# endernewton/tf-faster-rcnn

Measured on AMD Instinct MI355X. Metric: images/sec (600×1000) ResNet-101 Faster R-CNN at 1/2/4/8 MI355X, higher is better.
Workload: dtype f32 (operands, accumulators, results; GEMMs with Cin, Cout % 128 == 0 form each f32 product from two-piece fp16 operands with an exact power-of-two scale per 128-k block on the fp16 matrix pipe -- 3 MFMAs / product, dropped terms <= 3 * 2^-22, measured error vs float64 below the f32-MFMA kernel's; o

## Files before the change

tf-faster-rcnn_amd/csrc/gemm_h2.hip:

```cpp
#include "h2_common.h"
#include <mutex>
#include <type_traits>

typedef float f32x16 __attribute__((ext_vector_type(16)));
typedef _Float16 h8 __attribute__((ext_vector_type(8)));

#define LDS_AS __attribute__((address_space(3)))

struct GemmH2Params {
  const unsigned short* x; const float* x_inv; const unsigned short* w; const float* w_inv;
  const float* bias; const float* res; const unsigned short* resp; const float* resp_inv; float* y; unsigned short* yp; float* y_inv;
  int M, N, K, batch, act, nsteps, mtiles, ntiles;
  long long Mtot;
  int wshare;
  const float* mask;
  float* mean_part; int mean_rows;
#ifdef FRCNN_H2_TRACE
  unsigned long long* trace;
#endif
};

__device__ __forceinline__ void h2_glds16(unsigned voff, const void* sbase, unsigned lds_base) {
  unsigned keep;
  asm volatile(
// ... 12 lines not shown
  asm volatile(
      "s_mov_b32 %0, m0\n\t"
      "s_mov_b32 m0, %3\n\t"
      "s_nop 0\n\t"
      "global_load_lds_dword %1, %2\n\t"
      "s_mov_b32 m0, %0"
      : "=&s"(keep)
      : "v"(voff), "s"(sbase), "s"(lds_base)
      : "memory");
}

__device__ __forceinline__ void h2_glds16c(unsigned voff, const void* sbase, unsigned lds_base) {
  asm volatile(
      "s_mov_b32 m0, %2\n\t"
      "s_nop 0\n\t"
      "global_load_lds_dwordx4 %0, %1"
      :
      : "v"(voff), "s"(sbase), "s"(lds_base)
      : "memory");
}
__device__ __forceinline__ void h2_glds4c(unsigned voff, const void* sbase, unsigned lds_base) {
  asm volatile(
      "s_mov_b32 m0, %2\n\t"
      "s_nop 0\n\t"
      "global_load_lds_dword %0, %1"
      :
      : "v"(voff), "s"(sbase), "s"(lds_base)
      : "memory");
}

template <int N>
__device__ __forceinline__ void h2_wait_vmcnt() {
  asm volatile("s_waitcnt vmcnt(%0)" ::"n"(N) : "memory");
}

template <int BM, int BN, int WM, int WN, int NS, int WPE = 2, int TUNE = 0>
__global__ __launch_bounds__((BM / WM) * (BN / WN) * 64) __attribute__((amdgpu_waves_per_eu(WPE))) void k_gemm_h2(const GemmH2Params p) {
  constexpr int NW = (BM / WM) * (BN / WN);
  constexpr int TM = WM / 32, TN = WN / 32;
  constexpr int LA = 2 * BM / 16 / NW;
  constexpr int LB = 2 * BN / 16 / NW;
  constexpr int G = LA + LB;
  constexpr int SL = BM / 64;
  constexpr int XP = BM * 64, WP = BN * 64;
  constexpr bool PP = (TUNE & 32) != 0;
  constexpr bool LTB = (TUNE & 256) != 0;
  constexpr bool W21 = (TUNE & 512) != 0;
  constexpr bool DE = (TUNE & 1024) != 0;
  constexpr int NTA = (TUNE & 16384) ? 2 : 0;
  constexpr int S_OFF = 2 * XP + 2 * WP, STAGE = S_OFF + (PP ? 0 : 1024);
  constexpr int RED_OFF = NS * STAGE;
  constexpr int S2_OFF = RED_OFF + (BN / WN) * BM * 4;
  constexpr int CB_OFF = S2_OFF + (PP ? NW * 512 : (TUNE & 2) ? 2048 : 0);
  static_assert(!LTB || (!PP && NS == 2 && NW >= 3 && BN % 64 == 0), "light boundary: the two-slot one-barrier-per-slab schedule");
  static_assert(!DE || (LTB && W21 && BN == H2_KB), "deferred epilogue: built on the light boundary's LDS constants and counted waits");
  static_assert(!PP || (NW == 8 && NS == 3 && (TUNE & 2) && ((BM == 256 && WM == 64) || (BM == 128 && WM == 32)) && BN == 128 && WN == 64),
                "ping-pong geometry: 8 waves as 4 (M) x 2 (N), waves 0-3 = the upper half of the rows");
  static_assert((2 * BM / 16) % NW == 0 && (2 * BN / 16) % NW == 0, "tile/wave mismatch");
  static_assert(BM <= 256 && NS >= 2 && NS <= 4, "stage layout");
  static_assert((NS - 2) * (G + SL) <= 63, "vmcnt range");
  extern __shared__ __attribute__((aligned(16))) char smem[];

  const int tid = threadIdx.x, lane = tid & 63;
  const int wave = __builtin_amdgcn_readfirstlane(tid >> 6);
  const int per = p.mtiles * p.ntiles, T = per * p.batch;
  const int xcd = blockIdx.x & 7, wx = blockIdx.x >> 3, W8 = gridDim.x >> 3;
  const int tq = T / 8, tr = T % 8, tn = tq + (xcd < tr ? 1 : 0);
  const int t_end = (xcd < tr ? xcd * (tq + 1) : tr * (tq + 1) + (xcd - tr) * tq) + tn;
  const int tile0 = t_end - tn + wx;
  if (tile0 >= t_end) return;
  const int my_tiles = (t_end - tile0 + W8 - 1) / W8;
  int left = __builtin_amdgcn_readfirstlane(my_tiles * p.nsteps);

  const int wmi = wave / (BN / WN), wni = wave % (BN / WN);
  const int wm0 = wmi * WM, wn0 = wni * WN;
  const int frow = lane & 31, khalf = lane >> 5;

  const size_t xplane = (size_t)p.Mtot * p.K * 2, wplane = (size_t)p.N * p.K * 2;
  unsigned a_off[LA], b_off[LB], s_off[SL];
  const char* i_xb = nullptr; const char* i_wb = nullptr; const char* i_sb = nullptr;
  int i_tile = tile0, i_step = 0, i_par = 0, c_par = 0;
  int i_g = 0, i_bn0 = 0, i_cpar = 0, c_cpar = 0;
  int pend = 0;
#pragma unroll
  for (int t = 0; t < LB; ++t) {
    const int u = wave * LB + t, plane = u / (BN / 16), row = (u % (BN / 16)) * 16 + (lane >> 2), pos = lane & 3;
    b_off[t] = (unsigned)((size_t)plane * wplane + (size_t)row * p.K * 2 + ((pos ^ ((row >> ((TUNE & 8) ? 1 : 2)) & 3)) * 16));
// ... 212 lines not shown
#pragma unroll
      for (int i = 0; i < TM; ++i)
#pragma unroll
        for (int j = 0; j < TN; ++j) {
          tmp[i][j] = __builtin_amdgcn_mfma_f32_32x32x16_f16(wh[j], xl[i], tmp[i][j], 0, 0, 0);
          after(t * 3 * TM * TN + 2 * TM * TN + i * TN + j);
        }
    }
  };

  int c_tile = tile0, c_step = 0, cur = 0, nxt = 0;
  int c_bm0 = 0, c_bn0 = 0, c_g = 0;
  auto set_ctile = [&](int tl) {
    int g, mt, nt;
    tile_coords(tl, g, mt, nt);
    c_bm0 = mt * BM; c_bn0 = nt * BN; c_g = g;
  };
  const float act_lo = p.act == FRCNN_ACT_NONE ? -__builtin_inff() : 0.f;
  const float act_hi = p.act == FRCNN_ACT_RELU6 ? 6.f : __builtin_inff();

  auto rsrc_f = [&](const void* base, long long elems_left, int esize) {
    const long long bytes = elems_left * esize;
    return __builtin_amdgcn_make_buffer_rsrc((void*)base, 0, (int)max(0ll, min(bytes, 0x7fffffffll)), 0x00020000);
  };

  struct TileRef { int bm0, bn0, g, cpar; };
  auto ent_rsrc = [&](const void* base, int g, int esize) {
    const char* b = (const char*)base + (size_t)g * p.M * p.N * esize;
    return __builtin_amdgcn_make_buffer_rsrc((void*)b, 0, p.M * p.N * esize, 0x00020000);
  };
  const int lo4 = (frow * p.N + 4 * khalf) * 4;
  auto lo2_of = [&]() { int v = lo4; asm volatile("" : "+v"(v)); return v >> 1; };
  auto lo2w_of = [&]() { int v = lo4; asm volatile("" : "+v"(v)); return (v >> 1) + 8 * (int)(threadIdx.x >> 5 & 1); };
  auto sub_off = [&](const auto& T, int i, int j) {
    return __builtin_amdgcn_readfirstlane((T.bm0 + wm0 + i * 32) * p.N + T.bn0 + wn0 + j * 32);
  };

#ifdef FRCNN_H2_TRACE
  int tr_slab = 0;
  auto stamp = [&](int point) {
    if (p.trace && blockIdx.x < 16 && tr_slab < 64 && lane == 0)
      p.trace[(((size_t)blockIdx.x * NW + wave) * 64 + tr_slab) * 8 + point] = __builtin_amdgcn_s_memtime();
  };
  int tr_tile = 0;
  auto bstamp = [&](int point) {
    if (p.trace && blockIdx.x < 16 && tr_tile < 32 && lane == 0)
      p.trace[(size_t)16 * 8 * 64 * 8 + (((size_t)blockIdx.x * NW + wave) * 32 + tr_tile) * 8 + point] = __builtin_amdgcn_s_memtime();
  };
#else
  auto stamp = [](int) {};
  auto bstamp = [](int) {};
#endif
  float rri[TM];
  (void)rri;
  auto load_res_raw = [&](int i) {
    typedef unsigned u32x4 __attribute__((ext_vector_type(4)));
    const TileRef C{c_bm0, c_bn0, c_g, c_cpar};
    const bool planes = !p.res && p.resp;
    const auto none = __builtin_amdgcn_make_buffer_rsrc((void*)nullptr, 0, 0, 0x00020000);
    const auto r_even = p.res ? ent_rsrc(p.res, c_g, 4) : planes ? ent_rsrc(p.resp, c_g, 2) : none;
    const auto r_odd = p.res ? r_even : planes ? ent_rsrc(p.resp + (size_t)p.Mtot * p.N, c_g, 2) : none;
    const int step_q = planes ? 0 : 32, step_p = planes ? 32 : 0;
    int base = lo4;
    asm volatile("" : "+v"(base));
    if (planes) base = (base >> 1) + 8 * (int)(threadIdx.x >> 5 & 1);
#pragma unroll
    for (int j = 0; j < TN; ++j) {
      const int vo = base + sub_off(C, i, j) * (planes ? 2 : 4);
#pragma unroll
      for (int q = 0; q < 4; ++q) {
        const u32x4 ld = __builtin_amdgcn_raw_buffer_load_b128((q & 1) ? r_odd : r_even, vo, q * step_q + (q >> 1) * step_p, NTA);
        tot[i][j][4 * q + 0] = __uint_as_float(ld[0]); tot[i][j][4 * q + 1] = __uint_as_float(ld[1]);
        tot[i][j][4 * q + 2] = __uint_as_float(ld[2]); tot[i][j][4 * q + 3] = __uint_as_float(ld[3]);
      }
      pend += 4;
    }
    if (p.resp) rri[i] = p.resp_inv[(size_t)(c_bn0 / H2_KB) * p.Mtot + (size_t)c_g * p.M + min(c_bm0 + wm0 + i * 32 + frow, p.M - 1)];
  };
  auto init_tot = [&]() {
    if constexpr (DE) return;
    const size_t row_base = (size_t)c_g * p.M;
    typedef unsigned u32x4 __attribute__((ext_vector_type(4)));
    if (p.res) {
#pragma unroll
      for (int i = 0; i < TM; ++i)
#pragma unroll
        for (int j = 0; j < TN; ++j) {
          const int m0 = c_bm0 + wm0 + i * 32, nc = c_bn0 + wn0 + j * 32;
          const auto rr = rsrc_f(p.res + (long long)(row_base + m0) * p.N + nc, (long long)(p.M - m0) * p.N - nc, 4);
#pragma unroll
          for (int q = 0; q < 4; ++q) {
            const u32x4 ld = __builtin_amdgcn_raw_buffer_load_b128(rr, (frow * p.N + 4 * khalf) * 4 + 32 * q, 0, 0);
            tot[i][j][4 * q + 0] = __uint_as_float(ld[0]); tot[i][j][4 * q + 1] = __uint_as_float(ld[1]);
            tot[i][j][4 * q + 2] = __uint_as_float(ld[2]); tot[i][j][4 * q + 3] = __uint_as_float(ld[3]);
          }
        }
      pend += TM * TN * 4;
    } else if (p.resp) {
      float ri[TM];
#pragma unroll
      for (int i = 0; i < TM; ++i)
        ri[i] = p.resp_inv[(size_t)(c_bn0 / H2_KB) * p.Mtot + row_base + min(c_bm0 + wm0 + i * 32 + frow, p.M - 1)];
      h4 hv[TM][TN][4], lv[TM][TN][4];
#pragma unroll
      for (int i = 0; i < TM; ++i)
#pragma unroll
        for (int j = 0; j < TN; ++j) {
          const int m0 = c_bm0 + wm0 + i * 32, nc = c_bn0 + wn0 + j * 32;
          const long long sbase = (long long)(row_base + m0) * p.N + nc, left_e = (long long)(p.M - m0) * p.N - nc;
          const auto rh = rsrc_f(p.resp + sbase, left_e, 2), rl = rsrc_f(p.resp + (size_t)p.Mtot * p.N + sbase, left_e, 2);
// ... 60 lines not shown
      const int n0 = T.bn0 + wn0 + j * 32 + 4 * khalf;
#pragma unroll
      for (int q = 0; q < 4; ++q) {
        const float4 wi = LTB ? *(const float4*)(smem + CB_OFF + T.cpar * (2 * BN * 4) + (wn0 + j * 32 + 4 * khalf + 8 * q) * 4)
                             : *(const float4*)(p.w_inv + (size_t)(p.wshare ? 0 : T.g) * p.N + n0 + 8 * q);
#pragma unroll
        for (int i = 0; i < TM; ++i) {
          tot[i][j][4 * q + 0] = act_clamp(tot[i][j][4 * q + 0] * wi.x, act_lo, act_hi);
          tot[i][j][4 * q + 1] = act_clamp(tot[i][j][4 * q + 1] * wi.y, act_lo, act_hi);
          tot[i][j][4 * q + 2] = act_clamp(tot[i][j][4 * q + 2] * wi.z, act_lo, act_hi);
          tot[i][j][4 * q + 3] = act_clamp(tot[i][j][4 * q + 3] * wi.w, act_lo, act_hi);
        }
      }
    }
  };
  auto ep_mask = [&](const TileRef& T) {
    if ((TUNE & 128) && p.mask) {
      const auto rk = ent_rsrc(p.mask, T.g, 4);
#pragma unroll
      for (int i = 0; i < TM; ++i)
#pragma unroll
        for (int j = 0; j < TN; ++j) {
          const int vo = lo4 + sub_off(T, i, j) * 4;
          typedef unsigned u32x4 __attribute__((ext_vector_type(4)));
          u32x4 k[4];
#pragma unroll
          for (int q = 0; q < 4; ++q) k[q] = __builtin_amdgcn_raw_buffer_load_b128(rk, vo + 32 * q, 0, 0);
#pragma unroll
          for (int q = 0; q < 4; ++q)
#pragma unroll
            for (int e = 0; e < 4; ++e) tot[i][j][4 * q + e] = __uint_as_float(k[q][e]) > 0.f ? tot[i][j][4 * q + e] : 0.f;
        }
      pend += TM * TN * 4;
    }
  };
  auto ep_mean = [&](const TileRef& T) {
    const int nblk = (p.M + 31) >> 5;
#pragma unroll
    for (int i = 0; i < TM; ++i) {
      const int mb = T.bm0 + wm0 + i * 32;
      if (mb >= p.M) continue;
      const int m = mb + frow, g0 = mb / p.mean_rows, gid = m / p.mean_rows;
      const bool in_a = m < p.M && gid == g0, in_b = m < p.M && gid == g0 + 1;
      float* dst = p.mean_part + ((size_t)T.g * nblk + (mb >> 5)) * 2 * p.N;
#pragma unroll
      for (int j = 0; j < TN; ++j) {
        const int n0 = T.bn0 + wn0 + j * 32 + 4 * khalf;
#pragma unroll
        for (int q = 0; q < 4; ++q) {
          float a[4], b[4];
#pragma unroll
          for (int e = 0; e < 4; ++e) {
            const float v = tot[i][j][4 * q + e];
            a[e] = in_a ? v : 0.f;
            b[e] = in_b ? v : 0.f;
          }
#pragma unroll
          for (int o = 1; o < 32; o <<= 1)
#pragma unroll
            for (int e = 0; e < 4; ++e) {
              a[e] += __shfl_xor(a[e], o, 64);
              b[e] += __shfl_xor(b[e], o, 64);
            }
          if (frow == 0) {
            *(float4*)(dst + n0 + 8 * q) = make_float4(a[0], a[1], a[2], a[3]);
            *(float4*)(dst + p.N + n0 + 8 * q) = make_float4(b[0], b[1], b[2], b[3]);
          }
          pend += 2;
        }
      }
    }
  };
  auto ep_store_f32 = [&](const TileRef& T, int i) {
    if (!p.y) return;
    const auto ry = ent_rsrc(p.y, T.g, 4);
#pragma unroll
    for (int j = 0; j < TN; ++j) {
      const int lo = lo4 + sub_off(T, i, j) * 4;
#pragma unroll
      for (int q = 0; q < 4; ++q) {
        typedef unsigned u32x4 __attribute__((ext_vector_type(4)));
        u32x4 o;
        o[0] = __float_as_uint(tot[i][j][4 * q + 0]); o[1] = __float_as_uint(tot[i][j][4 * q + 1]);
        o[2] = __float_as_uint(tot[i][j][4 * q + 2]); o[3] = __float_as_uint(tot[i][j][4 * q + 3]);
        __builtin_amdgcn_raw_buffer_store_b128(o, ry, lo + 32 * q, 0, NTA);
      }
      pend += 4;
      if constexpr (DE) __builtin_amdgcn_sched_barrier(0);
    }
  };
  auto ep_rowmax_write = [&](float (&mx)[TM]) {
    float* red = (float*)(smem + RED_OFF);
#pragma unroll
    for (int i = 0; i < TM; ++i) {
      float m = 0.f;
#pragma unroll
      for (int j = 0; j < TN; ++j)
#pragma unroll
        for (int r = 0; r < 16; ++r) m = fmaxf(m, fabsf(tot[i][j][r]));
      m = fmaxf(m, __shfl_xor(m, 32, 64));
      mx[i] = m;
      if (BN / WN > 1 && khalf == 0) red[wni * BM + wm0 + i * 32 + frow] = m;
    }
  };
  auto ep_rowmax_merge = [&](float (&mx)[TM]) {
    const float* red = (const float*)(smem + RED_OFF);
#pragma unroll
    for (int i = 0; i < TM; ++i)
#pragma unroll
      for (int o = 0; o < BN / WN; ++o) mx[i] = fmaxf(mx[i], red[o * BM + wm0 + i * 32 + frow]);
  };
  auto ep_store_planes = [&](const TileRef& T, int i, float mxi) {
    const size_t row_base = (size_t)T.g * p.M;
    const size_t yplane = (size_t)p.Mtot * p.N;
    float scale, inv;
    h2_block_scale(mxi, scale, inv);
    const int m0 = T.bm0 + wm0 + i * 32;
    if (wni == 0 && khalf == 0 && m0 + frow < p.M)
      p.y_inv[(size_t)(T.bn0 / H2_KB) * p.Mtot + row_base + m0 + frow] = inv;
    const auto rh = ent_rsrc(p.yp, T.g, 2), rl = ent_rsrc(p.yp + yplane, T.g, 2);
#pragma unroll
    for (int j = 0; j < TN; ++j) {
      const int so = sub_off(T, i, j) * 2;
      typedef unsigned u32x2 __attribute__((ext_vector_type(2)));
      if constexpr (W21) {
        const int lo = lo2w_of() + so;
#pragma unroll
        for (int pq = 0; pq < 2; ++pq) {
          h4 ha, la, hb, lb;
          h2_split4(make_float4(tot[i][j][8 * pq + 0], tot[i][j][8 * pq + 1], tot[i][j][8 * pq + 2], tot[i][j][8 * pq + 3]), scale, ha, la);
          h2_split4(make_float4(tot[i][j][8 * pq + 4], tot[i][j][8 * pq + 5], tot[i][j][8 * pq + 6], tot[i][j][8 * pq + 7]), scale, hb, lb);
          const u32x2 uha = __builtin_bit_cast(u32x2, ha), uhb = __builtin_bit_cast(u32x2, hb);
          const u32x2 ula = __builtin_bit_cast(u32x2, la), ulb = __builtin_bit_cast(u32x2, lb);
          typedef unsigned u32x4 __attribute__((ext_vector_type(4)));
          const auto h0 = __builtin_amdgcn_permlane32_swap(uha[0], uhb[0], false, false), h1 = __builtin_amdgcn_permlane32_swap(uha[1], uhb[1], false, false);
          const auto l0 = __builtin_amdgcn_permlane32_swap(ula[0], ulb[0], false, false), l1 = __builtin_amdgcn_permlane32_swap(ula[1], ulb[1], false, false);
          __builtin_amdgcn_raw_buffer_store_b128(u32x4{h0[0], h1[0], h0[1], h1[1]}, rh, lo + 32 * pq, 0, NTA);
          __builtin_amdgcn_raw_buffer_store_b128(u32x4{l0[0], l1[0], l0[1], l1[1]}, rl, lo + 32 * pq, 0, NTA);
        }
        pend += 4;
        if constexpr (DE) __builtin_amdgcn_sched_barrier(0);
      } else {
        const int lo = lo2_of() + so;
#pragma unroll
        for (int q = 0; q < 4; ++q) {
          h4 hh, ll;
          h2_split4(make_float4(tot[i][j][4 * q + 0], tot[i][j][4 * q + 1], tot[i][j][4 * q + 2], tot[i][j][4 * q + 3]), scale, hh, ll);
          __builtin_amdgcn_raw_buffer_store_b64(__builtin_bit_cast(u32x2, hh), rh, lo + 16 * q, 0, 0);
          __builtin_amdgcn_raw_buffer_store_b64(__builtin_bit_cast(u32x2, ll), rl, lo + 16 * q, 0, 0);
        }
        pend += 8;
      }
// ... 20 lines not shown
      if (BN / WN > 1) {
        asm volatile("s_waitcnt lgkmcnt(0)" ::: "memory");
        __builtin_amdgcn_s_barrier();
        ep_rowmax_merge(mx);
      }
      bstamp(3);
#pragma unroll
      for (int i = 0; i < TM; ++i) ep_store_planes(T, i, mx[i]);
      bstamp(4);
      if (BN / WN > 1) {
        asm volatile("s_waitcnt lgkmcnt(0)" ::: "memory");
        __builtin_amdgcn_s_barrier();
      }
    }
    bstamp(5);
    c_cpar ^= 1;
  };

  constexpr int HALF = (TM + 1) / 2;
  bool have_prev = false;
  TileRef P{0, 0, 0, 0};
  float dmx[TM];
  (void)dmx;
  auto de_piece = [&](auto pos_c) {
    constexpr int POS = decltype(pos_c)::value;
    if constexpr (POS == 0) {
      if (have_prev) {
        ep_scale_act(P);
        ep_mask(P);
        if (p.yp) ep_rowmax_write(dmx);
      }
    } else if constexpr (POS == 1 || POS == 2) {
      constexpr int I0 = POS == 1 ? 0 : HALF, I1 = POS == 1 ? HALF : TM;
      if (have_prev) {
        if (POS == 1 && p.yp && BN / WN > 1) ep_rowmax_merge(dmx);
#pragma unroll
        for (int i = I0; i < I1; ++i) {
          ep_store_f32(P, i);
          if (p.yp) ep_store_planes(P, i, dmx[i]);
        }
      }
#pragma unroll
      for (int i = I0; i < I1; ++i) load_res_raw(i);
    }
  };

  auto slab = [&](auto pos_c, bool fold, bool first_block) {
    constexpr int POS = decltype(pos_c)::value;
    const std::integral_constant<bool, POS == 0> first_c{};
    stamp(0);
    if constexpr (DE) asm volatile("s_waitcnt lgkmcnt(0)" ::: "memory");
    if constexpr (LTB) {
      wait_pending(pend);
    } else if (left >= 1) {
      if (wave == 0) h2_wait_vmcnt<(NS - 2) * (G + SL)>(); else h2_wait_vmcnt<(NS - 2) * G>();
    } else {
      h2_wait_vmcnt<0>();
    }
    stamp(1);
    __builtin_amdgcn_s_barrier();
    stamp(2);
    const bool more = left > 0;
    constexpr int HALF = NO_LOAD ? 0 : (TUNE & 4) ? 0 : (TUNE & 1) ? (G + SL) / 2 : G + SL;
    static_assert(!LTB || NO_LOAD || HALF == G + SL, "light boundary: the slab's loads are issued in one burst");
    if (more) {
#pragma unroll
      for (int t = 0; t < HALF; ++t) issue_one(nxt, t);
      if constexpr (LTB) {
        if (i_step == 0) issue_cb();
        pend = 0;
      }
    }
    stamp(3);
    if constexpr (DE) {
      __builtin_amdgcn_sched_barrier(0);
      if (first_block) de_piece(pos_c);
      __builtin_amdgcn_sched_barrier(0);
    }
    float ainv[TM];
    if (fold) {
      const int soff = (TUNE & 2) ? S2_OFF + c_par * 1024 : cur * STAGE + S_OFF;
#pragma unroll
      for (int i = 0; i < TM; ++i) ainv[i] = *(const float*)(smem + soff + (wm0 + i * 32 + frow) * 4);
      c_par ^= 1;
    }
    if (!(TUNE & 4)) {
      slab_mfma(cur, first_c, [&]() {
        stamp(4);
        if (more && !NO_LOAD) {
#pragma unroll
          for (int t = HALF; t < G + SL; ++t) issue_one(nxt, t);
        }
      }, [](int) {});
    } else if (more) {
      slab_mfma(cur, first_c, []() {}, [&](int m) {
#pragma unroll
        for (int d = 0; d < ND; ++d)
          if (1 + (d * (NM - 1)) / ND == m) issue_one(nxt, d);
      });
    } else {
      slab_mfma(cur, first_c, []() {}, [](int) {});
    }
    stamp(5);
    if (more) {
      issue_advance();
      nxt = nxt + 1 == NS ? 0 : nxt + 1;
    }
    if (fold) {
      if (LTB && first_block) {
        const float* cbp = (const float*)(smem + CB_OFF + c_cpar * (2 * BN * 4));
        if (DE && !p.res && p.resp) {
          typedef unsigned u32x2 __attribute__((ext_vector_type(2)));
#pragma unroll
          for (int i = 0; i < TM; ++i)
#pragma unroll
            for (int j = 0; j < TN; ++j)
#pragma unroll
              for (int pq = 0; pq < 2; ++pq) {
                unsigned w[8];
#pragma unroll
                for (int e = 0; e < 8; ++e) w[e] = __float_as_uint(tot[i][j][8 * pq + e]);
                const auto h0 = __builtin_amdgcn_permlane32_swap(w[0], w[2], false, false), h1 = __builtin_amdgcn_permlane32_swap(w[1], w[3], false, false);
                const auto l0 = __builtin_amdgcn_permlane32_swap(w[4], w[6], false, false), l1 = __builtin_amdgcn_permlane32_swap(w[5], w[7], false, false);
                const h4 ha = __builtin_bit_cast(h4, u32x2{h0[0], h1[0]}), hb = __builtin_bit_cast(h4, u32x2{h0[1], h1[1]});
                const h4 la = __builtin_bit_cast(h4, u32x2{l0[0], l1[0]}), lb = __builtin_bit_cast(h4, u32x2{l0[1], l1[1]});
#pragma unroll
                for (int e = 0; e < 4; ++e) {
                  tot[i][j][8 * pq + e] = ((float)ha[e] + (float)la[e]) * rri[i];
                  tot[i][j][8 * pq + 4 + e] = ((float)hb[e] + (float)lb[e]) * rri[i];
                }
              }
        }
#pragma unroll
        for (int j = 0; j < TN; ++j)
#pragma unroll
          for (int q = 0; q < 4; ++q) {
            const float4 wi = *(const float4*)(cbp + wn0 + j * 32 + 4 * khalf + 8 * q);
            const float4 bv = p.bias ? *(const float4*)(cbp + BN + wn0 + j * 32 + 4 * khalf + 8 * q) : make_float4(0.f, 0.f, 0.f, 0.f);
            const float s0 = __uint_as_float(0x7f000000u - __float_as_uint(wi.x)), s1 = __uint_as_float(0x7f000000u - __float_as_uint(wi.y));
            const float s2 = __uint_as_float(0x7f000000u - __float_as_uint(wi.z)), s3 = __uint_as_float(0x7f000000u - __float_as_uint(wi.w));
#pragma unroll
            for (int i = 0; i < TM; ++i) {
              tot[i][j][4 * q + 0] = __builtin_fmaf(tmp[i][j][4 * q + 0], ainv[i], (tot[i][j][4 * q + 0] + bv.x) * s0);
              tot[i][j][4 * q + 1] = __builtin_fmaf(tmp[i][j][4 * q + 1], ainv[i], (tot[i][j][4 * q + 1] + bv.y) * s1);
              tot[i][j][4 * q + 2] = __builtin_fmaf(tmp[i][j][4 * q + 2], ainv[i], (tot[i][j][4 * q + 2] + bv.z) * s2);
              tot[i][j][4 * q + 3] = __builtin_fmaf(tmp[i][j][4 * q + 3], ainv[i], (tot[i][j][4 * q + 3] + bv.w) * s3);
            }
          }
      } else {
#pragma unroll
        for (int i = 0; i < TM; ++i)
#pragma unroll
          for (int j = 0; j < TN; ++j)
#pragma unroll
            for (int r = 0; r < 16; ++r) tot[i][j][r] = __builtin_fmaf(tmp[i][j][r], ainv[i], tot[i][j][r]);
      }
    }
    cur = cur + 1 == NS ? 0 : cur + 1;
    stamp(6);
#ifdef FRCNN_H2_TRACE
    ++tr_slab;
#endif
  };

  set_tile(i_tile);
  set_ctile(c_tile);
  if constexpr (PP) {
    const int grp = wave >> 2;
    h8 fxh[2][TM], fxl[2][TM], fwh[2][TN], fwl[2][TN];
    auto seg_barrier = [&]() {
      __builtin_amdgcn_sched_barrier(0);
      __builtin_amdgcn_s_barrier();
      __builtin_amdgcn_sched_barrier(0);
    };
    auto fold = [&]() {
      float ainv[TM];
#pragma unroll
      for (int i = 0; i < TM; ++i) ainv[i] = *(const float*)(smem + S2_OFF + (wave * 2 + c_par) * 256 + (i * 32 + frow) * 4);
      c_par ^= 1;
#pragma unroll
      for (int i = 0; i < TM; ++i)
#pragma unroll
        for (int j = 0; j < TN; ++j)
#pragma unroll
          for (int r = 0; r < 16; ++r) tot[i][j][r] = __builtin_fmaf(tmp[i][j][r], ainv[i], tot[i][j][r]);
    };
    auto pp_mem = [&](auto pos_c, bool fold_prev) -> bool {
      constexpr int POS = decltype(pos_c)::value;
      const char* sb = smem + cur * STAGE;
      stamp(0);
#pragma unroll
      for (int t = 0; t < 2; ++t) {
#pragma unroll
        for (int j = 0; j < TN; ++j) {
          const char* q = sb + w_row + j * 32 * 64 + (((2 * t + khalf) ^ sw) * 16);
          fwh[t][j] = __builtin_bit_cast(h8, *(const uint4*)(q));
          fwl[t][j] = __builtin_bit_cast(h8, *(const uint4*)(q + WP));
        }
#pragma unroll
        for (int i = 0; i < TM; ++i) {
          const char* q = sb + x_row + i * 32 * 64 + (((2 * t + khalf) ^ sw) * 16);
          fxh[t][i] = __builtin_bit_cast(h8, *(const uint4*)(q));
          fxl[t][i] = __builtin_bit_cast(h8, *(const uint4*)(q + XP));
        }
      }
      const bool more = left > 0;
      if (more) {
#pragma unroll
        for (int t = 0; t <= G; ++t) issue_one(nxt, t);
        issue_advance();
        nxt = nxt + 1 == NS ? 0 : nxt + 1;
      }
      if (fold_prev) fold();
      stamp(1);
      if (grp == 1) {
        if (more) h2_wait_vmcnt<(POS == 2 ? G + 1 : G)>(); else h2_wait_vmcnt<0>();
      }
      asm volatile("s_waitcnt lgkmcnt(0)" ::: "memory");
      stamp(2);
      seg_barrier();
      stamp(3);
      return more;
    };
    auto pp_mfma = [&](auto pos_c, bool issued) {
      constexpr int POS = decltype(pos_c)::value;
      __builtin_amdgcn_s_setprio(1);
#pragma unroll
      for (int t = 0; t < 2; ++t) {
#pragma unroll
        for (int i = 0; i < TM; ++i)
#pragma unroll
          for (int j = 0; j < TN; ++j) {
            if (POS == 0 && t == 0) {
              f32x16 z;
#pragma unroll
              for (int r = 0; r < 16; ++r) z[r] = 0.f;
              tmp[i][j] = __builtin_amdgcn_mfma_f32_32x32x16_f16(fwh[t][j], fxh[t][i], z, 0, 0, 0);
            } else {
              tmp[i][j] = __builtin_amdgcn_mfma_f32_32x32x16_f16(fwh[t][j], fxh[t][i], tmp[i][j], 0, 0, 0);
            }
          }
#pragma unroll
        for (int i = 0; i < TM; ++i)
#pragma unroll
          for (int j = 0; j < TN; ++j) tmp[i][j] = __builtin_amdgcn_mfma_f32_32x32x16_f16(fwl[t][j], fxh[t][i], tmp[i][j], 0, 0, 0);
#pragma unroll
        for (int i = 0; i < TM; ++i)
#pragma unroll
          for (int j = 0; j < TN; ++j) tmp[i][j] = __builtin_amdgcn_mfma_f32_32x32x16_f16(fwh[t][j], fxl[t][i], tmp[i][j], 0, 0, 0);
      }
      __builtin_amdgcn_s_setprio(0);
      stamp(4);
      if (grp == 0) {
        if (issued) h2_wait_vmcnt<(POS == 2 ? G + 1 : G)>(); else h2_wait_vmcnt<0>();
      }
      cur = cur + 1 == NS ? 0 : cur + 1;
      stamp(5);
      seg_barrier();
      stamp(6);
#ifdef FRCNN_H2_TRACE
      ++tr_slab;
#endif
    };
    bool two = false;
#pragma unroll
    for (int s2 = 0; s2 < 2; ++s2) {
      if (left > 0) {
#pragma unroll
        for (int t = 0; t <= G; ++t) issue_one(nxt, t);
        issue_advance();
        nxt = nxt + 1 == NS ? 0 : nxt + 1;
        two = s2 == 1;
      }
    }
    if (two) h2_wait_vmcnt<G>(); else h2_wait_vmcnt<0>();
    seg_barrier();
    if (grp == 1) seg_barrier();
    const int nkb = p.nsteps >> 2;
    for (int tl = 0; tl < my_tiles; ++tl) {
      init_tot();
      for (int kb = 0; kb < nkb; ++kb) {
        bool is;
        is = pp_mem(std::integral_constant<int, 0>{}, kb > 0); pp_mfma(std::integral_constant<int, 0>{}, is);
        is = pp_mem(std::integral_constant<int, 1>{}, false);  pp_mfma(std::integral_constant<int, 1>{}, is);
        is = pp_mem(std::integral_constant<int, 2>{}, false);  pp_mfma(std::integral_constant<int, 2>{}, is);
        is = pp_mem(std::integral_constant<int, 3>{}, false);  pp_mfma(std::integral_constant<int, 3>{}, is);
      }
      fold();
      epilogue();
      c_tile += W8;
      if (tl + 1 < my_tiles) set_ctile(c_tile);
    }
    if (grp == 0) seg_barrier();
    h2_wait_vmcnt<0>();
    return;
  }
#pragma unroll
  for (int s = 0; s < NS - 1; ++s) {
    if (left > 0) {
#pragma unroll
      for (int t = 0; t < G + SL; ++t) issue_one(nxt, t);
      if constexpr (LTB) {
        if (i_step == 0) issue_cb();
        pend = 0;
      }
      issue_advance();
      nxt = nxt + 1 == NS ? 0 : nxt + 1;
    }
  }
  const int nkb = p.nsteps >> 2;
  for (int tl = 0; tl < my_tiles; ++tl) {
    init_tot();
    bstamp(6);
#ifdef FRCNN_H2_TRACE
    ++tr_tile;
#endif
    for (int kb = 0; kb < nkb; ++kb) {
      slab(std::integral_constant<int, 0>{}, false, kb == 0);
      slab(std::integral_constant<int, 1>{}, false, kb == 0);
      slab(std::integral_constant<int, 2>{}, false, kb == 0);
      slab(std::integral_constant<int, 3>{}, true, kb == 0);
// ... 73 lines not shown
unsigned long long* g_h2_trace = nullptr;
extern "C" void frcnn_h2_set_trace(unsigned long long* buf) { g_h2_trace = buf; }
#endif

extern "C" size_t frcnn_h2_planes_bytes(long long rows, int K) {
  if (rows <= 0 || K <= 0) return 0;
  return (size_t)2 * (size_t)rows * (size_t)K * sizeof(unsigned short);
}

extern "C" int frcnn_h2_pack_w(const float* w_d, int G, int N, int K, void* planes_d, float* w_inv_d, void* stream) {
  if (!w_d || !planes_d || !w_inv_d || G <= 0 || N <= 0 || K <= 0) return FRCNN_E_ARG;
  if (K % 4) return FRCNN_E_UNSUPPORTED;
  const int rows = G * N;
  hipLaunchKernelGGL(k_h2_pack_w, dim3((unsigned)cdiv(rows, 4)), dim3(256), 0, (hipStream_t)stream, w_d, rows, N, K, (unsigned short*)planes_d, w_inv_d);
  LAUNCH_CHECK();
  return FRCNN_OK;
}

extern "C" int frcnn_h2_split(const float* x_d, long long M, int K, void* planes_d, float* inv_d, void* stream) {
  if (!x_d || !planes_d || !inv_d || M <= 0 || K <= 0) return FRCNN_E_ARG;
  if (K % H2_KB) return FRCNN_E_UNSUPPORTED;
  const long long pairs = M * (K / H2_KB);
  const unsigned grid = (unsigned)min((pairs + 7) / 8, (long long)256 * 64);
  hipLaunchKernelGGL(k_h2_split, dim3(grid), dim3(256), 0, (hipStream_t)stream, x_d, M, K, (unsigned short*)planes_d, inv_d);
  LAUNCH_CHECK();
  return FRCNN_OK;
}

template <int BM, int BN, int WM, int WN, int NS, int WPE = 2, int TUNE = 0>
static int launch_h2(const GemmH2Params& q, hipStream_t st) {
  constexpr int NT = (BM / WM) * (BN / WN) * 64;
  constexpr size_t lds = ((TUNE & 32) ? (size_t)NS * (2 * BM * 64 + 2 * BN * 64) + (size_t)(BN / WN) * BM * 4 + (size_t)(NT / 64) * 512
                                      : (size_t)NS * (2 * BM * 64 + 2 * BN * 64 + 1024) + (size_t)(BN / WN) * BM * 4 + ((TUNE & 2) ? 2048 : 0)) +
                         ((TUNE & 256) ? (size_t)2 * 2 * BN * 4 : 0);
  auto kern = k_gemm_h2<BM, BN, WM, WN, NS, WPE, TUNE>;
  static KernelOnce once;
  int slots = 0;
  HIP_TRY(kernel_once(once, (const void*)kern, NT, lds, &slots));
  if (slots < 8 || q.N % BN) return FRCNN_E_UNSUPPORTED;
  if (q.yp && BN != H2_KB) return FRCNN_E_UNSUPPORTED;
  GemmH2Params p = q;
  p.mtiles = cdiv(p.M, BM); p.ntiles = p.N / BN; p.nsteps = p.K / 32;
  const long long T = (long long)p.mtiles * p.ntiles * p.batch;
  if (T >= (1ll << 30)) return FRCNN_E_UNSUPPORTED;
  const int grid = (int)min((long long)(slots / 8) * 8, ((T + 7) / 8) * 8);
  hipLaunchKernelGGL(kern, dim3(grid), dim3(NT), lds, st, p);
  LAUNCH_CHECK();
  return FRCNN_OK;
}

static int run_h2(GemmH2Params& p, int cfg, hipStream_t st);

extern "C" int frcnn_gemm_h2(const void* x_planes_d, const float* x_inv_d, const void* w_planes_d, const float* w_inv_d, const float* bias_d,
                             const float* res_d, const void* res_planes_d, const float* res_inv_d, float* y_d, void* y_planes_d, float* y_inv_d,
                             int G, int M, int N, int K, int act, int cfg, void* stream) {
  if (!x_planes_d || !x_inv_d || !w_planes_d || !w_inv_d || (!y_d && !y_planes_d) || (y_planes_d && !y_inv_d) || G <= 0 || M <= 0 || N <= 0 ||
      K <= 0 || act < 0 || act > 2 || (res_d && res_planes_d) || (res_planes_d && !res_inv_d))
    return FRCNN_E_ARG;
  const long long Mtot = (long long)G * M;
  if (K % H2_KB || N % 128 || 4ll * Mtot * K >= (1ll << 32) || 4ll * N * K >= (1ll << 32) ||
      (long long)M * N >= (1ll << 29))
    return FRCNN_E_UNSUPPORTED;
  GemmH2Params p;
  p.x = (const unsigned short*)x_planes_d; p.x_inv = x_inv_d; p.w = (const unsigned short*)w_planes_d; p.w_inv = w_inv_d;
  p.bias = bias_d; p.res = res_d; p.resp = (const unsigned short*)res_planes_d; p.resp_inv = res_inv_d; p.y = y_d; p.yp = (unsigned short*)y_planes_d; p.y_inv = y_inv_d;
  p.M = M; p.N = N; p.K = K; p.batch = G; p.act = act; p.Mtot = Mtot;
  p.nsteps = p.mtiles = p.ntiles = 0;
// ... 6 lines not shown

extern "C" int frcnn_gemm_h2_masked(const void* x_planes_d, const float* x_inv_d, const void* w_planes_d, const float* w_inv_d, const float* bias_d,
                                    const float* res_d, const float* mask_d, float* y_d, void* y_planes_d, float* y_inv_d, int G, int M, int N, int K,
                                    int act, int cfg, void* stream) {
  if (!x_planes_d || !x_inv_d || !w_planes_d || !w_inv_d || !mask_d || (!y_d && !y_planes_d) || (y_planes_d && !y_inv_d) || G <= 0 || M <= 0 ||
      N <= 0 || K <= 0 || act < 0 || act > 2)
    return FRCNN_E_ARG;
  const long long Mtot = (long long)G * M;
  if (K % H2_KB || N % 128 || 4ll * Mtot * K >= (1ll << 32) || 4ll * N * K >= (1ll << 32) || (long long)M * N >= (1ll << 29)) return FRCNN_E_UNSUPPORTED;
  GemmH2Params p;
  p.x = (const unsigned short*)x_planes_d; p.x_inv = x_inv_d; p.w = (const unsigned short*)w_planes_d; p.w_inv = w_inv_d;
  p.bias = bias_d; p.res = res_d; p.resp = nullptr; p.resp_inv = nullptr; p.y = y_d; p.yp = (unsigned short*)y_planes_d; p.y_inv = y_inv_d;
  p.M = M; p.N = N; p.K = K; p.batch = G; p.act = act; p.Mtot = Mtot;
  p.nsteps = p.mtiles = p.ntiles = 0;
#ifdef FRCNN_H2_TRACE
  p.trace = g_h2_trace;
#endif
  p.mean_part = nullptr; p.mean_rows = 0; p.wshare = 0; p.mask = mask_d;
  return run_h2(p, cfg, (hipStream_t)stream);
}

static int run_h2(GemmH2Params& p, int cfg, hipStream_t st) {
  const int G = p.batch, M = p.M, N = p.N, K = p.K;
  if (cfg < 0) {
    const long long mt256 = (M + 255) / 256;
#ifndef FRCNN_H2_PP_MIN_K
#define FRCNN_H2_PP_MIN_K 1024
#endif
    const int pp_min_k = ((cfg == -4 || cfg == -5 || cfg == -6) && !p.mean_part) ? 512 : FRCNN_H2_PP_MIN_K;
    const int pp_cfg = (cfg == -3 || cfg == -4 || (cfg == -6 && K < FRCNN_H2_PP_MIN_K)) ? 34 : 21;
    const bool pp = K >= pp_min_k && mt256 * 256 * 100 <= (long long)M * 104 && mt256 * (N / 128) * G >= 256;
    const bool tiny = (long long)((M + 127) / 128) * (N / 128) * G < 150;
    const bool de = cfg != -2 && cfg != -7 && !p.mean_part && !p.mask && ((p.resp && p.yp && !p.y) || cfg == -8);
    cfg = pp ? pp_cfg : tiny ? (cfg == -2 ? 12 : (de && cfg == -8) ? 41 : 33) : (cfg == -2 ? 9 : de ? 40 : 31);
  }
  if (p.mean_part && (cfg == 40 || cfg == 41)) cfg = cfg == 40 ? 31 : 33;
  if (p.mask) switch (cfg) {
    case 9: return launch_h2<128, 128, 64, 64, 2, 2, 2 + 128>(p, st);
    case 12: return launch_h2<64, 128, 32, 64, 2, 2, 128>(p, st);
    case 21: return launch_h2<256, 128, 64, 64, 3, 2, 34 + 128>(p, st);
    case 30: return launch_h2<128, 128, 64, 64, 2, 2, 2 + 256 + 128>(p, st);
    case 31: return launch_h2<128, 128, 64, 64, 2, 2, 2 + 256 + 512 + 128>(p, st);
    case 32: return launch_h2<128, 128, 64, 64, 2, 2, 2 + 512 + 128>(p, st);
    case 33: return launch_h2<64, 128, 32, 64, 2, 2, 256 + 512 + 128>(p, st);
    case 34: return launch_h2<256, 128, 64, 64, 3, 2, 34 + 512 + 128>(p, st);
    case 40: return launch_h2<128, 128, 64, 64, 2, 2, 2 + 256 + 512 + 1024 + 128>(p, st);
    case 41: return launch_h2<64, 128, 32, 64, 2, 2, 256 + 512 + 1024 + 128>(p, st);
    default: return FRCNN_E_ARG;
  }
  switch (cfg) {
    case 9: return launch_h2<128, 128, 64, 64, 2, 2, 2>(p, st);
    case 12: return launch_h2<64, 128, 32, 64, 2>(p, st);
    case 21: return launch_h2<256, 128, 64, 64, 3, 2, 34>(p, st);
    case 30: return launch_h2<128, 128, 64, 64, 2, 2, 2 + 256>(p, st);
    case 31: return launch_h2<128, 128, 64, 64, 2, 2, 2 + 256 + 512>(p, st);
    case 32: return launch_h2<128, 128, 64, 64, 2, 2, 2 + 512>(p, st);
    case 33: return launch_h2<64, 128, 32, 64, 2, 2, 256 + 512>(p, st);
    case 34: return launch_h2<256, 128, 64, 64, 3, 2, 34 + 512>(p, st);
    case 40: return launch_h2<128, 128, 64, 64, 2, 2, 2 + 256 + 512 + 1024>(p, st);
    case 41: return launch_h2<64, 128, 32, 64, 2, 2, 256 + 512 + 1024>(p, st);
#ifdef FRCNN_ABLATION
    case 0: return launch_h2<128, 128, 64, 64, 2>(p, st);
    case 1: return launch_h2<128, 128, 64, 64, 3>(p, st);
    case 2: return launch_h2<128, 128, 64, 64, 4>(p, st);
    case 3: return launch_h2<256, 128, 64, 64, 2>(p, st);
    case 8: return launch_h2<128, 128, 64, 64, 2, 2, 1>(p, st);
    case 13: return launch_h2<64, 128, 32, 64, 3>(p, st);
    case 15: return launch_h2<64, 128, 32, 64, 4>(p, st);
    case 14: return launch_h2<128, 128, 64, 64, 2, 2, 4>(p, st);
    case 18: return launch_h2<128, 128, 64, 64, 2, 2, 10>(p, st);
    case 24: return launch_h2<128, 128, 32, 64, 3, 2, 34>(p, st);
    case 22: return launch_h2<256, 128, 64, 64, 3, 2, 34 + 64>(p, st);
    case 23: return launch_h2<128, 128, 64, 64, 2, 2, 2 + 64>(p, st);
    case 20: return launch_h2<128, 128, 64, 64, 2, 2, 18>(p, st);
    case 42: return launch_h2<128, 128, 64, 64, 2, 2, 2 + 256 + 512 + 1024 + 16384>(p, st);
    case 43: return launch_h2<128, 128, 64, 64, 2, 2, 2 + 256 + 512 + 1024 + 32768>(p, st);
    case 44: return launch_h2<128, 128, 64, 64, 2, 2, 2 + 256 + 512 + 1024 + 16384 + 32768>(p, st);
    case 50: return launch_h2<128, 128, 64, 64, 2, 2, 2 + 256 + 512 + 2048>(p, st);
    case 51: return launch_h2<128, 128, 64, 64, 2, 2, 2 + 256 + 512 + 4096>(p, st);
    case 52: return launch_h2<128, 128, 64, 64, 2, 2, 2 + 256 + 512 + 8192>(p, st);
    case 53: return launch_h2<128, 128, 64, 64, 2, 2, 2 + 256 + 512 + 2048 + 4096>(p, st);
    case 54: return launch_h2<128, 128, 64, 64, 2, 2, 2 + 256 + 512 + 4096 + 8192>(p, st);
    case 55: return launch_h2<128, 128, 64, 64, 2, 2, 2 + 256 + 512 + 2048 + 4096 + 8192>(p, st);
#endif
    default: return FRCNN_E_ARG;
  }
}

__global__ __launch_bounds__(256) void k_h2_mean_finish(const float* __restrict__ part, int G, int M, int N4, int rows, float4* __restrict__ out) {
  const long long t = (long long)blockIdx.x * blockDim.x + threadIdx.x;
  const int per = M / rows;
  if (t >= (long long)G * per * N4) return;
  const int n4 = (int)(t % N4);
// ... 47 lines not shown
```

Before: 539.9.

## Extend ping-pong GEMM schedule with light boundary and deferred epilogue, route mid-K shapes

Ports the light-boundary first-fold and the deferred epilogue into the 8-wave ping-pong GEMM schedule. Per-row inverse scales now go through LDS via async global-to-LDS loads, vmcnt waits become runtime-counted through a binary dispatch over immediate waits, and the previous tile's epilogue is spread across the next tile's memory phases. The heuristic also routes K in [512,1024) shapes to the ping-pong config 34. Two new configs (45, 46) are added but not selected by default. The change adds LDS use, register pressure and complex wait accounting, which raises correctness and occupancy risk.

```diff
diff --git a/tf-faster-rcnn_amd/csrc/gemm_h2.hip b/tf-faster-rcnn_amd/csrc/gemm_h2.hip
--- a/tf-faster-rcnn_amd/csrc/gemm_h2.hip
+++ b/tf-faster-rcnn_amd/csrc/gemm_h2.hip
@@ -68,6 +68,16 @@
 template <int N>
 __device__ __forceinline__ void h2_wait_vmcnt() {
   asm volatile("s_waitcnt vmcnt(%0)" ::"n"(N) : "memory");
+}
+
+template <int LO, int HI>
+__device__ __forceinline__ void h2_wait_vmcnt_le(int n) {
+  if constexpr (LO == HI) {
+    h2_wait_vmcnt<LO>();
+  } else {
+    constexpr int MID = (LO + HI + 1) / 2;
+    if (n >= MID) h2_wait_vmcnt_le<MID, HI>(n); else h2_wait_vmcnt_le<LO, MID - 1>(n);
+  }
 }
 
 template <int BM, int BN, int WM, int WN, int NS, int WPE = 2, int TUNE = 0>
@@ -88,7 +98,8 @@
   constexpr int RED_OFF = NS * STAGE;
   constexpr int S2_OFF = RED_OFF + (BN / WN) * BM * 4;
   constexpr int CB_OFF = S2_OFF + (PP ? NW * 512 : (TUNE & 2) ? 2048 : 0);
-  static_assert(!LTB || (!PP && NS == 2 && NW >= 3 && BN % 64 == 0), "light boundary: the two-slot one-barrier-per-slab schedule");
+  constexpr int RRI_OFF = CB_OFF + (LTB ? 2 * 2 * BN * 4 : 0);
+  static_assert(!LTB || ((PP || NS == 2) && NW >= 3 && BN % 64 == 0), "light boundary: the two-slot one-barrier-per-slab or the ping-pong schedule");
   static_assert(!DE || (LTB && W21 && BN == H2_KB), "deferred epilogue: built on the light boundary's LDS constants and counted waits");
   static_assert(!PP || (NW == 8 && NS == 3 && (TUNE & 2) && ((BM == 256 && WM == 64) || (BM == 128 && WM == 32)) && BN == 128 && WN == 64),
                 "ping-pong geometry: 8 waves as 4 (M) x 2 (N), waves 0-3 = the upper half of the rows");
@@ -367,6 +378,7 @@
   const int lo4 = (frow * p.N + 4 * khalf) * 4;
   auto lo2_of = [&]() { int v = lo4; asm volatile("" : "+v"(v)); return v >> 1; };
   auto lo2w_of = [&]() { int v = lo4; asm volatile("" : "+v"(v)); return (v >> 1) + 8 * (int)(threadIdx.x >> 5 & 1); };
+  auto frow_at_use = [&]() { int v = (int)(threadIdx.x & 31); if constexpr (PP && DE) asm volatile("" : "+v"(v)); return v; };
   auto sub_off = [&](const auto& T, int i, int j) {
     return __builtin_amdgcn_readfirstlane((T.bm0 + wm0 + i * 32) * p.N + T.bn0 + wn0 + j * 32);
   };
@@ -410,7 +422,16 @@
       }
       pend += 4;
     }
-    if (p.resp) rri[i] = p.resp_inv[(size_t)(c_bn0 / H2_KB) * p.Mtot + (size_t)c_g * p.M + min(c_bm0 + wm0 + i * 32 + frow, p.M - 1)];
+    if constexpr (PP) {
+      if (p.resp && i == 0) {
+        h2_glds4c((unsigned)(min(c_bm0 + wm0 + lane, p.M - 1) * 4),
+                  uniform_ptr((const char*)(p.resp_inv + (size_t)(c_bn0 / H2_KB) * p.Mtot + (size_t)c_g * p.M)),
+                  __builtin_amdgcn_readfirstlane(lds0 + RRI_OFF + wave * 256));
+        pend += 1;
+      }
+    } else if (p.resp) {
+      rri[i] = p.resp_inv[(size_t)(c_bn0 / H2_KB) * p.Mtot + (size_t)c_g * p.M + min(c_bm0 + wm0 + i * 32 + frow_at_use(), p.M - 1)];
+    }
   };
   auto init_tot = [&]() {
     if constexpr (DE) return;
@@ -537,6 +558,42 @@
             for (int e = 0; e < 4; ++e) tot[i][j][4 * q + e] = __uint_as_float(k[q][e]) > 0.f ? tot[i][j][4 * q + e] : 0.f;
         }
       pend += TM * TN * 4;
+    }
+  };
+  auto ep_mean_row = [&](const TileRef& T, int i) {
+    const int nblk = (p.M + 31) >> 5;
+    {
+      const int mb = T.bm0 + wm0 + i * 32;
+      if (mb >= p.M) return;
+      const int fr = frow_at_use(), m = mb + fr, g0 = mb / p.mean_rows, gid = m / p.mean_rows;
+      const bool in_a = m < p.M && gid == g0, in_b = m < p.M && gid == g0 + 1;
+      float* dst = p.mean_part + ((size_t)T.g * nblk + (mb >> 5)) * 2 * p.N;
+#pragma unroll
+      for (int j = 0; j < TN; ++j) {
+        const int n0 = T.bn0 + wn0 + j * 32 + 4 * khalf;
+#pragma unroll
+        for (int q = 0; q < 4; ++q) {
+          float a[4], b[4];
+#pragma unroll
+          for (int e = 0; e < 4; ++e) {
+            const float v = tot[i][j][4 * q + e];
+            a[e] = in_a ? v : 0.f;
+            b[e] = in_b ? v : 0.f;
+          }
+#pragma unroll
+          for (int o = 1; o < 32; o <<= 1)
+#pragma unroll
+            for (int e = 0; e < 4; ++e) {
+              a[e] += __shfl_xor(a[e], o, 64);
+              b[e] += __shfl_xor(b[e], o, 64);
+            }
+          if (fr == 0) {
+            *(float4*)(dst + n0 + 8 * q) = make_float4(a[0], a[1], a[2], a[3]);
+            *(float4*)(dst + p.N + n0 + 8 * q) = make_float4(b[0], b[1], b[2], b[3]);
+          }
+          pend += 2;
+        }
+      }
     }
   };
   auto ep_mean = [&](const TileRef& T) {
@@ -576,6 +633,7 @@
       }
     }
   };
+
   auto ep_store_f32 = [&](const TileRef& T, int i) {
     if (!p.y) return;
     const auto ry = ent_rsrc(p.y, T.g, 4);
@@ -621,8 +679,9 @@
     float scale, inv;
     h2_block_scale(mxi, scale, inv);
     const int m0 = T.bm0 + wm0 + i * 32;
-    if (wni == 0 && khalf == 0 && m0 + frow < p.M)
-      p.y_inv[(size_t)(T.bn0 / H2_KB) * p.Mtot + row_base + m0 + frow] = inv;
+    const int fr = frow_at_use();
+    if (wni == 0 && khalf == 0 && m0 + fr < p.M)
+      p.y_inv[(size_t)(T.bn0 / H2_KB) * p.Mtot + row_base + m0 + fr] = inv;
     const auto rh = ent_rsrc(p.yp, T.g, 2), rl = ent_rsrc(p.yp + yplane, T.g, 2);
 #pragma unroll
     for (int j = 0; j < TN; ++j) {
@@ -709,7 +768,25 @@
       }
     } else if constexpr (POS == 1 || POS == 2) {
       constexpr int I0 = POS == 1 ? 0 : HALF, I1 = POS == 1 ? HALF : TM;
-      if (have_prev) {
+      if constexpr (PP) {
+        if (have_prev) {
+          if (p.mean_part) {
+#pragma unroll
+            for (int i = I0; i < I1; ++i) ep_mean_row(P, i);
+          }
+          const float* red = (const float*)(smem + RED_OFF);
+#pragma unroll
+          for (int i = I0; i < I1; ++i) {
+            ep_store_f32(P, i);
+            if (p.yp) {
+              float m = 0.f;
+#pragma unroll
+              for (int o = 0; o < BN / WN; ++o) m = fmaxf(m, red[o * BM + wm0 + i * 32 + frow]);
+              ep_store_planes(P, i, m);
+            }
+          }
+        }
+      } else if (have_prev) {
         if (POS == 1 && p.yp && BN / WN > 1) ep_rowmax_merge(dmx);
 #pragma unroll
         for (int i = I0; i < I1; ++i) {
@@ -720,6 +797,49 @@
 #pragma unroll
       for (int i = I0; i < I1; ++i) load_res_raw(i);
     }
+  };
+
+  auto fold_first = [&](const float (&ainv)[TM]) {
+    const float* cbp = (const float*)(smem + CB_OFF + c_cpar * (2 * BN * 4));
+    if (DE && !p.res && p.resp) {
+      typedef unsigned u32x2 __attribute__((ext_vector_type(2)));
+#pragma unroll
+      for (int i = 0; i < TM; ++i)
+#pragma unroll
+        for (int j = 0; j < TN; ++j)
+#pragma unroll
+          for (int pq = 0; pq < 2; ++pq) {
+            unsigned w[8];
+#pragma unroll
+            for (int e = 0; e < 8; ++e) w[e] = __float_as_uint(tot[i][j][8 * pq + e]);
+            const auto h0 = __builtin_amdgcn_permlane32_swap(w[0], w[2], false, false), h1 = __builtin_amdgcn_permlane32_swap(w[1], w[3], false, false);
+            const auto l0 = __builtin_amdgcn_permlane32_swap(w[4], w[6], false, false), l1 = __builtin_amdgcn_permlane32_swap(w[5], w[7], false, false);
+            const h4 ha = __builtin_bit_cast(h4, u32x2{h0[0], h1[0]}), hb = __builtin_bit_cast(h4, u32x2{h0[1], h1[1]});
+            const h4 la = __builtin_bit_cast(h4, u32x2{l0[0], l1[0]}), lb = __builtin_bit_cast(h4, u32x2{l0[1], l1[1]});
+#pragma unroll
+            for (int e = 0; e < 4; ++e) {
+              const float ri = PP ? *(const float*)(smem + RRI_OFF + wave * 256 + (i * 32 + frow) * 4) : rri[i];
+              tot[i][j][8 * pq + e] = ((float)ha[e] + (float)la[e]) * ri;
+              tot[i][j][8 * pq + 4 + e] = ((float)hb[e] + (float)lb[e]) * ri;
+            }
+          }
+    }
+#pragma unroll
+    for (int j = 0; j < TN; ++j)
+#pragma unroll
+      for (int q = 0; q < 4; ++q) {
+        const float4 wi = *(const float4*)(cbp + wn0 + j * 32 + 4 * khalf + 8 * q);
+        const float4 bv = p.bias ? *(const float4*)(cbp + BN + wn0 + j * 32 + 4 * khalf + 8 * q) : make_float4(0.f, 0.f, 0.f, 0.f);
+        const float s0 = __uint_as_float(0x7f000000u - __float_as_uint(wi.x)), s1 = __uint_as_float(0x7f000000u - __float_as_uint(wi.y));
+        const float s2 = __uint_as_float(0x7f000000u - __float_as_uint(wi.z)), s3 = __uint_as_float(0x7f000000u - __float_as_uint(wi.w));
+#pragma unroll
+        for (int i = 0; i < TM; ++i) {
+          tot[i][j][4 * q + 0] = __builtin_fmaf(tmp[i][j][4 * q + 0], ainv[i], (tot[i][j][4 * q + 0] + bv.x) * s0);
+          tot[i][j][4 * q + 1] = __builtin_fmaf(tmp[i][j][4 * q + 1], ainv[i], (tot[i][j][4 * q + 1] + bv.y) * s1);
+          tot[i][j][4 * q + 2] = __builtin_fmaf(tmp[i][j][4 * q + 2], ainv[i], (tot[i][j][4 * q + 2] + bv.z) * s2);
+          tot[i][j][4 * q + 3] = __builtin_fmaf(tmp[i][j][4 * q + 3], ainv[i], (tot[i][j][4 * q + 3] + bv.w) * s3);
+        }
+      }
   };
 
   auto slab = [&](auto pos_c, bool fold, bool first_block) {
@@ -785,45 +905,7 @@
     }
     if (fold) {
       if (LTB && first_block) {
-        const float* cbp = (const float*)(smem + CB_OFF + c_cpar * (2 * BN * 4));
-        if (DE && !p.res && p.resp) {
-          typedef unsigned u32x2 __attribute__((ext_vector_type(2)));
-#pragma unroll
-          for (int i = 0; i < TM; ++i)
-#pragma unroll
-            for (int j = 0; j < TN; ++j)
-#pragma unroll
-              for (int pq = 0; pq < 2; ++pq) {
-                unsigned w[8];
-#pragma unroll
-                for (int e = 0; e < 8; ++e) w[e] = __float_as_uint(tot[i][j][8 * pq + e]);
-                const auto h0 = __builtin_amdgcn_permlane32_swap(w[0], w[2], false, false), h1 = __builtin_amdgcn_permlane32_swap(w[1], w[3], false, false);
-                const auto l0 = __builtin_amdgcn_permlane32_swap(w[4], w[6], false, false), l1 = __builtin_amdgcn_permlane32_swap(w[5], w[7], false, false);
-                const h4 ha = __builtin_bit_cast(h4, u32x2{h0[0], h1[0]}), hb = __builtin_bit_cast(h4, u32x2{h0[1], h1[1]});
-                const h4 la = __builtin_bit_cast(h4, u32x2{l0[0], l1[0]}), lb = __builtin_bit_cast(h4, u32x2{l0[1], l1[1]});
-#pragma unroll
-                for (int e = 0; e < 4; ++e) {
-                  tot[i][j][8 * pq + e] = ((float)ha[e] + (float)la[e]) * rri[i];
-                  tot[i][j][8 * pq + 4 + e] = ((float)hb[e] + (float)lb[e]) * rri[i];
-                }
-              }
-        }
-#pragma unroll
-        for (int j = 0; j < TN; ++j)
-#pragma unroll
-          for (int q = 0; q < 4; ++q) {
-            const float4 wi = *(const float4*)(cbp + wn0 + j * 32 + 4 * khalf + 8 * q);
-            const float4 bv = p.bias ? *(const float4*)(cbp + BN + wn0 + j * 32 + 4 * khalf + 8 * q) : make_float4(0.f, 0.f, 0.f, 0.f);
-            const float s0 = __uint_as_float(0x7f000000u - __float_as_uint(wi.x)), s1 = __uint_as_float(0x7f000000u - __float_as_uint(wi.y));
-            const float s2 = __uint_as_float(0x7f000000u - __float_as_uint(wi.z)), s3 = __uint_as_float(0x7f000000u - __float_as_uint(wi.w));
-#pragma unroll
-            for (int i = 0; i < TM; ++i) {
-              tot[i][j][4 * q + 0] = __builtin_fmaf(tmp[i][j][4 * q + 0], ainv[i], (tot[i][j][4 * q + 0] + bv.x) * s0);
-              tot[i][j][4 * q + 1] = __builtin_fmaf(tmp[i][j][4 * q + 1], ainv[i], (tot[i][j][4 * q + 1] + bv.y) * s1);
-              tot[i][j][4 * q + 2] = __builtin_fmaf(tmp[i][j][4 * q + 2], ainv[i], (tot[i][j][4 * q + 2] + bv.z) * s2);
-              tot[i][j][4 * q + 3] = __builtin_fmaf(tmp[i][j][4 * q + 3], ainv[i], (tot[i][j][4 * q + 3] + bv.w) * s3);
-            }
-          }
+        fold_first(ainv);
       } else {
 #pragma unroll
         for (int i = 0; i < TM; ++i)
@@ -850,11 +932,14 @@
       __builtin_amdgcn_s_barrier();
       __builtin_amdgcn_sched_barrier(0);
     };
-    auto fold = [&]() {
-      float ainv[TM];
+    auto fold_ainv = [&](float (&ainv)[TM]) {
 #pragma unroll
       for (int i = 0; i < TM; ++i) ainv[i] = *(const float*)(smem + S2_OFF + (wave * 2 + c_par) * 256 + (i * 32 + frow) * 4);
       c_par ^= 1;
+    };
+    auto fold = [&]() __attribute__((always_inline)) {
+      float ainv[TM];
+      fold_ainv(ainv);
 #pragma unroll
       for (int i = 0; i < TM; ++i)
 #pragma unroll
@@ -862,10 +947,26 @@
 #pragma unroll
           for (int r = 0; r < 16; ++r) tot[i][j][r] = __builtin_fmaf(tmp[i][j][r], ainv[i], tot[i][j][r]);
     };
-    auto pp_mem = [&](auto pos_c, bool fold_prev) -> bool {
+    auto pp_fold_first = [&]() __attribute__((always_inline)) {
+      float ainv[TM];
+      fold_ainv(ainv);
+      fold_first(ainv);
+    };
+    auto pp_wait = [&](int n) {
+      h2_wait_vmcnt_le<0, 63>(__builtin_amdgcn_readfirstlane(min(n, 63)));
+    };
+    auto pp_mem = [&](auto pos_c, bool fold_prev, bool first_fold, bool drain) -> int {
       constexpr int POS = decltype(pos_c)::value;
       const char* sb = smem + cur * STAGE;
       stamp(0);
+      if constexpr (LTB) {
+        if (first_fold) pp_fold_first();
+      }
+      if constexpr (DE) {
+        __builtin_amdgcn_sched_barrier(0);
+        if (drain) de_piece(pos_c);
+        __builtin_amdgcn_sched_barrier(0);
+      }
 #pragma unroll
       for (int t = 0; t < 2; ++t) {
 #pragma unroll
@@ -882,24 +983,36 @@
         }
       }
       const bool more = left > 0;
+      int n = pend;
       if (more) {
+        const int batch = G + ((i_step & 3) == 0 ? 1 : 0);
 #pragma unroll
         for (int t = 0; t <= G; ++t) issue_one(nxt, t);
+        if constexpr (LTB) {
+          const int older = pend;
+          pend = 0;
+          if (i_step == 0) {
+            issue_cb();
+            pend = (wave == 1 ? BN / 64 : 0) + ((wave == 2 && p.bias) ? BN / 64 : 0);
+          }
+          n = older + batch + pend;
+        }
         issue_advance();
         nxt = nxt + 1 == NS ? 0 : nxt + 1;
       }
-      if (fold_prev) fold();
+      if (fold_prev && !first_fold) fold();
       stamp(1);
       if (grp == 1) {
-        if (more) h2_wait_vmcnt<(POS == 2 ? G + 1 : G)>(); else h2_wait_vmcnt<0>();
+        if constexpr (LTB) pp_wait(n);
+        else if (more) h2_wait_vmcnt<(POS == 2 ? G + 1 : G)>(); else h2_wait_vmcnt<0>();
       }
       asm volatile("s_waitcnt lgkmcnt(0)" ::: "memory");
       stamp(2);
       seg_barrier();
       stamp(3);
-      return more;
+      return LTB ? n : (more ? 1 : 0);
     };
-    auto pp_mfma = [&](auto pos_c, bool issued) {
+    auto pp_mfma = [&](auto pos_c, int issued) {
       constexpr int POS = decltype(pos_c)::value;
       __builtin_amdgcn_s_setprio(1);
 #pragma unroll
@@ -929,7 +1042,8 @@
       __builtin_amdgcn_s_setprio(0);
       stamp(4);
       if (grp == 0) {
-        if (issued) h2_wait_vmcnt<(POS == 2 ? G + 1 : G)>(); else h2_wait_vmcnt<0>();
+        if constexpr (LTB) pp_wait(issued);
+        else if (issued) h2_wait_vmcnt<(POS == 2 ? G + 1 : G)>(); else h2_wait_vmcnt<0>();
       }
       cur = cur + 1 == NS ? 0 : cur + 1;
       stamp(5);
@@ -945,6 +1059,9 @@
       if (left > 0) {
 #pragma unroll
         for (int t = 0; t <= G; ++t) issue_one(nxt, t);
+        if constexpr (LTB) {
+          if (i_step == 0) issue_cb();
+        }
         issue_advance();
         nxt = nxt + 1 == NS ? 0 : nxt + 1;
         two = s2 == 1;
@@ -957,13 +1074,24 @@
     for (int tl = 0; tl < my_tiles; ++tl) {
       init_tot();
       for (int kb = 0; kb < nkb; ++kb) {
-        bool is;
-        is = pp_mem(std::integral_constant<int, 0>{}, kb > 0); pp_mfma(std::integral_constant<int, 0>{}, is);
-        is = pp_mem(std::integral_constant<int, 1>{}, false);  pp_mfma(std::integral_constant<int, 1>{}, is);
-        is = pp_mem(std::integral_constant<int, 2>{}, false);  pp_mfma(std::integral_constant<int, 2>{}, is);
-        is = pp_mem(std::integral_constant<int, 3>{}, false);  pp_mfma(std::integral_constant<int, 3>{}, is);
-      }
-      fold();
+        const bool ff = LTB && kb == 1, dr = DE && kb == 0;
+        int is;
+        is = pp_mem(std::integral_constant<int, 0>{}, kb > 0, ff, dr); pp_mfma(std::integral_constant<int, 0>{}, is);
+        is = pp_mem(std::integral_constant<int, 1>{}, false, false, dr); pp_mfma(std::integral_constant<int, 1>{}, is);
+        is = pp_mem(std::integral_constant<int, 2>{}, false, false, dr); pp_mfma(std::integral_constant<int, 2>{}, is);
+        is = pp_mem(std::integral_constant<int, 3>{}, false, false, false); pp_mfma(std::integral_constant<int, 3>{}, is);
+      }
+      if (LTB && nkb == 1) pp_fold_first(); else fold();
+      if constexpr (DE) {
+        if (tl + 1 < my_tiles) {
+          P = TileRef{c_bm0, c_bn0, c_g, c_cpar};
+          have_prev = true;
+          c_cpar ^= 1;
+          c_tile += W8;
+          set_ctile(c_tile);
+          continue;
+        }
+      }
       epilogue();
       c_tile += W8;
       if (tl + 1 < my_tiles) set_ctile(c_tile);
@@ -1103,7 +1231,7 @@
   constexpr int NT = (BM / WM) * (BN / WN) * 64;
   constexpr size_t lds = ((TUNE & 32) ? (size_t)NS * (2 * BM * 64 + 2 * BN * 64) + (size_t)(BN / WN) * BM * 4 + (size_t)(NT / 64) * 512
                                       : (size_t)NS * (2 * BM * 64 + 2 * BN * 64 + 1024) + (size_t)(BN / WN) * BM * 4 + ((TUNE & 2) ? 2048 : 0)) +
-                         ((TUNE & 256) ? (size_t)2 * 2 * BN * 4 : 0);
+                         ((TUNE & 256) ? (size_t)2 * 2 * BN * 4 : 0) + (((TUNE & 32) && (TUNE & 1024)) ? (size_t)(NT / 64) * 256 : 0);
   auto kern = k_gemm_h2<BM, BN, WM, WN, NS, WPE, TUNE>;
   static KernelOnce once;
   int slots = 0;
@@ -1176,7 +1304,9 @@
     const bool pp = K >= pp_min_k && mt256 * 256 * 100 <= (long long)M * 104 && mt256 * (N / 128) * G >= 256;
     const bool tiny = (long long)((M + 127) / 128) * (N / 128) * G < 150;
     const bool de = cfg != -2 && cfg != -7 && !p.mean_part && !p.mask && ((p.resp && p.yp && !p.y) || cfg == -8);
-    cfg = pp ? pp_cfg : tiny ? (cfg == -2 ? 12 : (de && cfg == -8) ? 41 : 33) : (cfg == -2 ? 9 : de ? 40 : 31);
+    const bool pp_short = (cfg == -1 || cfg == -8) && !p.mask && !p.mean_part && K >= 512 && K < FRCNN_H2_PP_MIN_K &&
+                          mt256 * 256 * 100 <= (long long)M * 104 && mt256 * (N / 128) * G >= 256;
+    cfg = pp_short ? 34 : pp ? pp_cfg : tiny ? (cfg == -2 ? 12 : (de && cfg == -8) ? 41 : 33) : (cfg == -2 ? 9 : de ? 40 : 31);
   }
   if (p.mean_part && (cfg == 40 || cfg == 41)) cfg = cfg == 40 ? 31 : 33;
   if (p.mask) switch (cfg) {
@@ -1203,6 +1333,8 @@
     case 34: return launch_h2<256, 128, 64, 64, 3, 2, 34 + 512>(p, st);
     case 40: return launch_h2<128, 128, 64, 64, 2, 2, 2 + 256 + 512 + 1024>(p, st);
     case 41: return launch_h2<64, 128, 32, 64, 2, 2, 256 + 512 + 1024>(p, st);
+    case 45: return launch_h2<256, 128, 64, 64, 3, 2, 34 + 256 + 512 + 1024>(p, st);
+    case 46: return launch_h2<256, 128, 64, 64, 3, 2, 34 + 256 + 512>(p, st);
 #ifdef FRCNN_ABLATION
     case 0: return launch_h2<128, 128, 64, 64, 2>(p, st);
     case 1: return launch_h2<128, 128, 64, 64, 3>(p, st);
```

Measured after the change: 542.8 (median of 6 runs). No clear change (+0.5%).
